# iosefa/obia

Hardware: AMD Instinct MI355X
Metric: Mpixel/s (SLIC+zonal feats) on 16384²×8-band; achieved HBM GB/s fraction (higher is better)
Workload: dtype f32

## Files before the change

### obia_amd/_lib.py

```python
import ctypes
import os
import subprocess

import numpy as np

_CSRC = os.path.join(os.path.dirname(os.path.abspath(__file__)), "csrc")
LIB_PATH = os.environ.get("OBIA_HIP_LIB") or os.path.join(_CSRC, "libobia_hip.so")

OBIA_OK = 0
MASK_SEEDS_CHUNK = 1024
E_INVALID, E_HIP, E_NOMEM, E_UNSUPPORTED, E_EMPTY, E_NONFINITE = -1, -2, -3, -4, -5, -6


class SlicParams(ctypes.Structure):
    _fields_ = [("compactness", ctypes.c_double), ("min_size_factor", ctypes.c_double),
                ("max_size_factor", ctypes.c_double), ("n_segments", ctypes.c_int32),
                ("max_num_iter", ctypes.c_int32), ("convert2lab", ctypes.c_int32),
                ("enforce_connectivity", ctypes.c_int32), ("slic_zero", ctypes.c_int32),
                ("start_label", ctypes.c_int32), ("normalize_bands", ctypes.c_int32),
                ("exit_on_fixed_point", ctypes.c_int32), ("reserved", ctypes.c_int32),
                ("sigma_zyx", ctypes.c_double * 3), ("spacing_zyx", ctypes.c_double * 3)]


class SlicSeeds(ctypes.Structure):
# ... 159 lines not shown


def last_error():
    return load().obia_last_error().decode("utf-8", "replace")


def check(rc):
    if rc == OBIA_OK:
        return
    msg = last_error()
    if rc in (E_INVALID, E_EMPTY, E_NONFINITE):
        raise ValueError(msg)
    if rc == E_UNSUPPORTED:
        raise NotImplementedError(msg)
    if rc == E_NOMEM:
        raise MemoryError(msg)
    raise RuntimeError(f"obia_hip error {rc}: {msg}")


class Context:

    def __init__(self, device=0, stream=None):
        lib = load()
        if stream is None:
            self._h = lib.obia_create(int(device))
        else:
            self._h = lib.obia_create_on_stream(int(device), ctypes.c_void_p(int(stream)))
        if not self._h:
            raise RuntimeError(f"obia_create failed: {last_error()} (obia_amd needs an AMD GPU; there is no CPU path)")
        self.device = int(device)

    @property
    def handle(self):
        return self._h

    def close(self):
        if getattr(self, "_h", None):
            load().obia_destroy(self._h)
            self._h = None

    def __del__(self):
        try:
            self.close()
        except Exception:
            pass

    def set_profiling(self, on):
        check(load().obia_set_profiling(self._h, int(on)))

    def timing(self):
        lib = load()
        names = ["assign_ms", "sweeps", "features_ms", "connectivity_ms", "zonal_ms", "total_ms", "prepass_ms", "assign_px",
                 "prepass_px", "assign_store_px", "assign_busy_ms", "prepass_busy_ms", "batch_repeats",
                 "prepass_shared_px", "feature_fused_px", "prepass_group_launches", "fills", "uploads", "readbacks"]
        return {n: lib.obia_last_timing(self._h, i) for i, n in enumerate(names)}

    def workspace_bytes(self):
        return int(load().obia_workspace_bytes(self._h))


_default_ctx = {}


def default_context(device=0):
    ctx = _default_ctx.get(device)
    if ctx is None:
        ctx = _default_ctx[device] = Context(device)
    return ctx


def np_ptr(a):
    return None if a is None else ctypes.c_void_p(a.ctypes.data)


def mask_bytes(mask, device=None):
    import torch
    m = torch.as_tensor(mask, device=device)
    if m.dtype == torch.bool:
        m = m.contiguous().view(torch.uint8)
    elif m.dtype != torch.uint8:
        m = (m != 0).view(torch.uint8)
    return m.contiguous()
```

### obia_amd/csrc/common.hpp

```cpp
#pragma once
#include <hip/hip_runtime.h>
#include <algorithm>
#include <cstdint>
#include <cstdio>
#include <cstring>
#include <string>
#include <vector>

#include "../../include/obia_hip.h"

struct obia_ctx;

namespace obia {

void set_error(const char *fmt, ...);

#define OBIA_HIP_TRY(expr)                                                                       \
    do {                                                                                         \
        hipError_t e__ = (expr);                                                                 \
        if (e__ != hipSuccess) {                                                                 \
            obia::set_error("%s:%d: %s -> %s", __FILE__, __LINE__, #expr, hipGetErrorString(e__)); \
            return OBIA_E_HIP;                                                                   \
        }                                                                                        \
    } while (0)

#define OBIA_TRY(expr)            \
    do {                          \
        int rc__ = (expr);        \
        if (rc__ != OBIA_OK) return rc__; \
    } while (0)

class Arena {
  public:
    ~Arena() { release(); }
    void *alloc(size_t bytes);
    template <typename T> T *get(size_t n) { return static_cast<T *>(alloc(n * sizeof(T))); }
    void reset();
    void release();
    struct Mark { size_t block, used, total; };
    Mark mark() const;
    void rewind(const Mark &m);
    size_t capacity() const;
    bool failed() const { return failed_; }

  private:
    struct Block { char *p; size_t size; size_t used; };
    std::vector<Block> blocks_;
    size_t high_water_ = 0, cur_total_ = 0, cur_ = 0;
    bool failed_ = false;
};

class PlanBlob {
  public:
    template <typename T> T *add(obia_ctx *ctx, const T *host, size_t n) { return static_cast<T *>(add_bytes(ctx, host, n * sizeof(T))); }
    int flush(obia_ctx *ctx);
    void drop() { dev_ = host_ = nullptr; cap_ = used_ = 0; }
  private:
    void *add_bytes(obia_ctx *ctx, const void *host, size_t bytes);
    char *dev_ = nullptr, *host_ = nullptr;
    size_t cap_ = 0, used_ = 0;
};

struct Timing {
    double assign_ms = 0, prepass_ms = 0, feat_ms = 0, cc_ms = 0, zonal_ms = 0, total_ms = 0;
    double assign_px = 0, prepass_px = 0;
    double prepass_shared_px = 0;
    double assign_store_px = 0;
    double feat_fused_px = 0;
    int sweeps = 0;
    int prepass_group_launches = 0;
    int batch_repeats = 0;
    double assign_busy_ms = 0, prepass_busy_ms = 0;
    int fills = 0, uploads = 0, readbacks = 0;
};

}

struct obia_ctx {
    int device = 0;
    hipStream_t stream = nullptr;
    bool own_stream = false;
    obia::Arena arena;
    void *pinned = nullptr;
    size_t pinned_bytes = 0;
    unsigned long long *defer_buf = nullptr;
    bool defer_pending = false;
    double defer_shared_px = 0;
    int32_t *cc_visited = nullptr;
    size_t cc_visited_px = 0;
    bool cc_visited_dirty = false;
    char *up_buf = nullptr;
    size_t up_bytes = 0, up_used = 0;
    obia::PlanBlob plan;
    int profiling = 0;
    obia::Timing timing;
    struct Span { int kind; hipEvent_t a, b; };
    std::vector<Span> spans;
    std::vector<hipEvent_t> event_pool;
    size_t events_used = 0;
    hipStream_t side = nullptr;
    hipEvent_t aux_fork = nullptr, aux_join = nullptr;
    hipEvent_t grp_fork = nullptr, grp_join = nullptr;
    int spatial_residency[4] = {0, 0, 0, 0};
};

namespace obia {

enum TimeKind { T_ASSIGN = 0, T_FEAT = 2, T_CC = 3, T_ZONAL = 4, T_TOTAL = 5, T_PREPASS = 6 };

struct ScopedSpan {
    obia_ctx *ctx; bool on; size_t idx;
    ScopedSpan(obia_ctx *c, int kind);
    ~ScopedSpan();
};
struct KernelSpan {
    hipEvent_t a = nullptr, b = nullptr;
    KernelSpan(obia_ctx *c, int kind);
};
void begin_timing(obia_ctx *ctx);
void resolve_timing(obia_ctx *ctx);

int read_back(obia_ctx *ctx, void *host_dst, const void *dev_src, size_t bytes);
int upload_async(obia_ctx *ctx, void *dev_dst, const void *host_src, size_t bytes);
int fill_async(obia_ctx *ctx, void *dev_dst, int byte, size_t bytes);

struct ClearRange { void *p; unsigned long long bytes; unsigned value, pad; };
struct ClearTable { ClearRange r[16]; int n; };
class ClearSet {
  public:
    explicit ClearSet(obia_ctx *ctx) : ctx_(ctx) { t_.n = 0; }
    int add(void *dev, int byte, size_t bytes);
    int flush();
  private:
    obia_ctx *ctx_;
    ClearTable t_;
};

int side_stream(obia_ctx *ctx);
void debug_sync(obia_ctx *ctx, const char *stage);

static inline int cdiv(long long a, long long b) { return (int)((a + b - 1) / b); }
static inline unsigned flat_grid(long long n) { return (unsigned)std::max<long long>(1, std::min<long long>(cdiv(n, 256), 8192)); }


int enter(obia_ctx *ctx);

int quiesce(obia_ctx *ctx, int rc);

enum FrameOpts : unsigned { FRAME_PLAIN = 0, FRAME_TIMING = 1, FRAME_TOTAL = 2 | FRAME_TIMING };
void frame_begin(obia_ctx *ctx, unsigned opts);
int frame_end(obia_ctx *ctx, unsigned opts, int rc);
template <typename Body> int call_frame(obia_ctx *ctx, unsigned opts, Body &&body) {
    frame_begin(ctx, opts);
    int rc;
    if ((opts & FRAME_TOTAL) == FRAME_TOTAL) {
        ScopedSpan total(ctx, T_TOTAL);
        rc = body();
    } else {
        rc = body();
    }
    return frame_end(ctx, opts, rc);
}

class Staging {
  public:
    explicit Staging(obia_ctx *ctx) : ctx_(ctx) {}
    ~Staging() { (void)finish(); }
    Staging(const Staging &) = delete;
    Staging &operator=(const Staging &) = delete;
    template <typename T> T *in(const T *host, size_t n) { return static_cast<T *>(upload(host, n * sizeof(T))); }
// ... 25 lines not shown
```

### obia_amd/csrc/context.cpp

```cpp
#include "common.hpp"
#include "../../include/obia_testing.h"

#include <algorithm>
#include <cstdlib>
#include <utility>

#include <cstdarg>

namespace obia {

static thread_local std::string g_last_error;

void set_error(const char *fmt, ...) {
    char buf[1024];
    va_list ap;
    va_start(ap, fmt);
    vsnprintf(buf, sizeof(buf), fmt, ap);
    va_end(ap);
    g_last_error = buf;
}

void *Arena::alloc(size_t bytes) {
    bytes = (bytes + 255) & ~size_t(255);
    if (bytes == 0) bytes = 256;
// ... 49 lines not shown
    if (blocks_.size() > 1) {
        size_t total = 0;
        for (auto &b : blocks_) total += b.size;
        for (auto &b : blocks_) (void)hipFree(b.p);
        blocks_.clear();
        void *p = nullptr;
        if (hipMalloc(&p, high_water_ + (high_water_ >> 3)) == hipSuccess) blocks_.push_back(Block{static_cast<char *>(p), high_water_ + (high_water_ >> 3), 0});
        (void)total;
    } else if (!blocks_.empty()) {
        blocks_[0].used = 0;
    }
}

void Arena::release() {
    for (auto &b : blocks_) (void)hipFree(b.p);
    blocks_.clear();
}

size_t Arena::capacity() const {
    size_t t = 0;
    for (auto &b : blocks_) t += b.size;
    return t;
}

static hipEvent_t get_event(obia_ctx *ctx) {
    if (ctx->events_used == ctx->event_pool.size()) {
        hipEvent_t e = nullptr;
        (void)hipEventCreate(&e);
        ctx->event_pool.push_back(e);
    }
    return ctx->event_pool[ctx->events_used++];
}

ScopedSpan::ScopedSpan(obia_ctx *c, int kind) : ctx(c), on(c->profiling == 1 || (c->profiling == 2 && kind == T_ASSIGN)), idx(0) {
    if (!on) return;
    obia_ctx::Span s{kind, get_event(ctx), get_event(ctx)};
    (void)hipEventRecord(s.a, ctx->stream);
    idx = ctx->spans.size();
    ctx->spans.push_back(s);
}
ScopedSpan::~ScopedSpan() {
    if (on) (void)hipEventRecord(ctx->spans[idx].b, ctx->stream);
}

int side_stream(obia_ctx *ctx) {
    if (!ctx->aux_fork) OBIA_HIP_TRY(hipEventCreateWithFlags(&ctx->aux_fork, hipEventDisableTiming));
    if (!ctx->aux_join) OBIA_HIP_TRY(hipEventCreateWithFlags(&ctx->aux_join, hipEventDisableTiming));
    if (!ctx->grp_fork) OBIA_HIP_TRY(hipEventCreateWithFlags(&ctx->grp_fork, hipEventDisableTiming));
    if (!ctx->grp_join) OBIA_HIP_TRY(hipEventCreateWithFlags(&ctx->grp_join, hipEventDisableTiming));
    if (!ctx->side) OBIA_HIP_TRY(hipStreamCreateWithFlags(&ctx->side, hipStreamNonBlocking));
    return OBIA_OK;
}

KernelSpan::KernelSpan(obia_ctx *c, int kind) {
    if (!(c->profiling == 1 || (c->profiling == 2 && kind == T_ASSIGN))) return;
    a = get_event(c);
    b = get_event(c);
    c->spans.push_back(obia_ctx::Span{kind, a, b});
}

void begin_timing(obia_ctx *ctx) {
    ctx->spans.clear();
    ctx->events_used = 0;
    ctx->timing = Timing();
}

void resolve_timing(obia_ctx *ctx) {
    if (!ctx->profiling) return;
    (void)hipStreamSynchronize(ctx->stream);
    std::vector<std::pair<double, double>> iv[2];
    hipEvent_t ref = nullptr;
    for (auto &s : ctx->spans) {
        float ms = 0;
        if (hipEventElapsedTime(&ms, s.a, s.b) != hipSuccess) { (void)hipGetLastError(); continue; }
        if (s.kind == T_ASSIGN || s.kind == T_PREPASS) {
            if (!ref) ref = s.a;
            float end = 0;
            if (hipEventElapsedTime(&end, ref, s.b) == hipSuccess) iv[s.kind == T_ASSIGN ? 0 : 1].emplace_back((double)end - ms, (double)end);
            else (void)hipGetLastError();
        }
        switch (s.kind) {
            case T_ASSIGN: ctx->timing.assign_ms += ms; ctx->timing.sweeps += 1; break;
            case T_FEAT: ctx->timing.feat_ms += ms; break;
            case T_CC: ctx->timing.cc_ms += ms; break;
            case T_ZONAL: ctx->timing.zonal_ms += ms; break;
            case T_TOTAL: ctx->timing.total_ms += ms; break;
            case T_PREPASS: ctx->timing.prepass_ms += ms; break;
            default: break;
        }
    }
    for (int c = 0; c < 2; ++c) {
        std::sort(iv[c].begin(), iv[c].end());
        double busy = 0, lo = 0, hi = -1;
        for (auto &x : iv[c]) {
            if (hi < lo || x.first > hi) { if (hi > lo) busy += hi - lo; lo = x.first; hi = x.second; }
            else if (x.second > hi) hi = x.second;
        }
        if (hi > lo) busy += hi - lo;
        (c == 0 ? ctx->timing.assign_busy_ms : ctx->timing.prepass_busy_ms) += busy;
    }
    ctx->spans.clear();
}

int read_back(obia_ctx *ctx, void *host_dst, const void *dev_src, size_t bytes) {
    if (bytes > ctx->pinned_bytes) {
        if (ctx->pinned) (void)hipHostFree(ctx->pinned);
        ctx->pinned = nullptr;
        size_t want = bytes < 4096 ? 4096 : bytes;
        OBIA_HIP_TRY(hipHostMalloc(&ctx->pinned, want, hipHostMallocDefault));
        ctx->pinned_bytes = want;
    }
    OBIA_TRY(ctx->plan.flush(ctx));
    OBIA_HIP_TRY(hipMemcpyAsync(ctx->pinned, dev_src, bytes, hipMemcpyDeviceToHost, ctx->stream));
    ctx->timing.readbacks += 1;
    OBIA_HIP_TRY(hipStreamSynchronize(ctx->stream));
    ctx->up_used = 0;
    memcpy(host_dst, ctx->pinned, bytes);
    return OBIA_OK;
}

void debug_sync(obia_ctx *ctx, const char *stage) {
    static const bool on = std::getenv("OBIA_DEBUG_SYNC") != nullptr;
    if (!on) return;
    const hipError_t e = hipStreamSynchronize(ctx->stream);
    fprintf(stderr, "[obia debug] %s: %s\n", stage, e == hipSuccess ? "ok" : hipGetErrorString(e));
    fflush(stderr);
}

int fill_async(obia_ctx *ctx, void *dev_dst, int byte, size_t bytes) {
    if (bytes == 0) return OBIA_OK;
    OBIA_HIP_TRY(hipMemsetAsync(dev_dst, byte, bytes, ctx->stream));
    ctx->timing.fills += 1;
    return OBIA_OK;
}

template <bool RAGGED> __global__ __launch_bounds__(256) void clear_ranges_kernel(const ClearTable T) {
    const size_t tid = (size_t)blockIdx.x * blockDim.x + threadIdx.x, stride = (size_t)gridDim.x * blockDim.x;
    for (int k = 0; k < T.n; ++k) {
        unsigned char *p = static_cast<unsigned char *>(T.r[k].p);
        const size_t n = T.r[k].bytes;
        const unsigned v = (T.r[k].value & 0xffu) * 0x01010101u;
        size_t head = RAGGED ? (16 - (reinterpret_cast<uintptr_t>(p) & 15)) & 15 : 0;
        if (head > n) head = n;
        const size_t nvec = (n - head) / 16, tail0 = head + nvec * 16;
        uint4 *pv = reinterpret_cast<uint4 *>(p + head);
        for (size_t i = tid; i < nvec; i += stride) pv[i] = make_uint4(v, v, v, v);
        if (RAGGED) {
            if (tid < head) p[tid] = (unsigned char)v;
            if (tid < n - tail0) p[tail0 + tid] = (unsigned char)v;
        }
    }
}

// ... 245 lines not shown
        for (int i = 0; i < n; ++i) OBIA_TRY(clr.add(dev_ptrs[i], values[i], (size_t)bytes[i]));
        return clr.flush();
    });
}

int64_t obia_workspace_bytes(obia_ctx *ctx) { return ctx ? (int64_t)ctx->arena.capacity() : 0; }

void obia_slic_default_params(obia_slic_params *p) {
    if (!p) return;
    p->n_segments = 100;
    p->compactness = 10.0;
    p->max_num_iter = 10;
    p->convert2lab = -1;
    p->enforce_connectivity = 1;
    p->min_size_factor = 0.5;
    p->max_size_factor = 3.0;
    p->slic_zero = 0;
    p->start_label = 1;
    p->normalize_bands = 0;
    p->exit_on_fixed_point = 0;
    p->reserved = 0;
    p->sigma_zyx[0] = p->sigma_zyx[1] = p->sigma_zyx[2] = 0.0;
    p->spacing_zyx[0] = p->spacing_zyx[1] = p->spacing_zyx[2] = 1.0;
}

int obia_set_profiling(obia_ctx *ctx, int enabled) {
    if (!ctx) { set_error("null context"); return OBIA_E_INVALID; }
    ctx->profiling = enabled < 0 ? 0 : (enabled > 2 ? 1 : enabled);
    return OBIA_OK;
}

double obia_last_timing(obia_ctx *ctx, int what) {
    if (!ctx) return -1.0;
    switch (what) {
        case 0: return ctx->timing.assign_ms;
        case 1: return (double)ctx->timing.sweeps;
        case 2: return ctx->timing.feat_ms;
        case 3: return ctx->timing.cc_ms;
        case 4: return ctx->timing.zonal_ms;
        case 5: return ctx->timing.total_ms;
        case 6: return ctx->timing.prepass_ms;
        case 7: return ctx->timing.assign_px;
        case 8: return ctx->timing.prepass_px;
        case 9: return ctx->timing.assign_store_px;
        case 10: return ctx->timing.assign_busy_ms;
        case 11: return ctx->timing.prepass_busy_ms;
        case 12: return (double)ctx->timing.batch_repeats;
        case 13: return ctx->timing.prepass_shared_px;
        case 14: return ctx->timing.feat_fused_px;
        case 15: return (double)ctx->timing.prepass_group_launches;
        case 16: return (double)ctx->timing.fills;
        case 17: return (double)ctx->timing.uploads;
        case 18: return (double)ctx->timing.readbacks;
        default: return -1.0;
    }
}

}
```

### obia_amd/csrc/slic_sweep.hip

```cpp
#include "slic.hpp"
#include "slic_features.hpp"

#include <type_traits>
#include <hip/hip_ext.h>

#include <cstdlib>

namespace obia {

#ifdef OBIA_STAMP
__device__ unsigned long long g_tl[65536 * 4 * 24];
#define STAMP_DECL unsigned long long st_t = clock64(), st_t0 = st_t, st_r0 = __builtin_amdgcn_s_memrealtime(), st_acc[12] = {0, 0, 0, 0, 0, 0, 0, 0, 0, 0, 0, 0}, st_cnt[6] = {0, 0, 0, 0, 0, 0};
#define STAMP_COUNT(i, v) st_cnt[i] += (v);
#define STAMP(i) { const unsigned long long st_n = clock64(); st_acc[i] += st_n - st_t; st_t = st_n; }
#ifndef OBIA_STAMP_KIND
#define OBIA_STAMP_KIND 0
#endif
#define STAMP_FLUSH if (accumulate && (LEAN ? 1 : 0) == OBIA_STAMP_KIND && (threadIdx.x & 63) == 0 && gtile < 65536) { unsigned long long *st_o = g_tl + ((size_t)gtile * 4 + (threadIdx.x >> 6)) * 24; for (int st_i = 0; st_i < 12; ++st_i) st_o[st_i] = st_acc[st_i]; st_o[12] = st_t0; st_o[13] = clock64(); st_o[14] = st_r0; st_o[15] = __builtin_amdgcn_s_memrealtime(); for (int st_i = 0; st_i < 6; ++st_i) st_o[16 + st_i] = st_cnt[st_i]; }
#else
#define STAMP_DECL
#define STAMP(i)
#define STAMP_COUNT(i, v)
#define STAMP_FLUSH
#endif
// ... 1096 lines not shown
    slic_assign_body<CP, MASKED, false, false, false, false, true, NCH>(OBIA_ASSIGN_ARGS, nullptr);
}

template <int CP, bool MASKED, bool FIXPT>
__global__ __launch_bounds__(NT) __attribute__((amdgpu_waves_per_eu(LEAN_WAVES, LEAN_WAVES))) void slic_prepass_kernel(OBIA_ASSIGN_PARAMS, const int *__restrict__ act_tiles) {
    slic_assign_body<CP, MASKED, true, FIXPT, false, true, false>(OBIA_ASSIGN_ARGS, act_tiles);
}

#include "slic_spatial.hip"

#ifdef OBIA_STAMP
extern "C" void obia_debug_timeline(unsigned long long *out, int nwaves) {
    (void)hipMemcpyFromSymbol(out, HIP_SYMBOL(g_tl), sizeof(unsigned long long) * 24 * (size_t)nwaves);
}
#endif

template <int CP, bool MASKED>
__global__ __launch_bounds__(256) void slic_maxdist_kernel(const SlicProblem *__restrict__ probs, const float *__restrict__ feat,
                                                           const uint8_t *__restrict__ mask, const int32_t *__restrict__ labels,
                                                           float *__restrict__ cent, int start_label, int nch) {
    constexpr int RS = CENT_REC + CP;
    const SlicProblem P = probs[blockIdx.y];
    for (int y = blockIdx.x; y < P.H; y += gridDim.x)
        for (int x = threadIdx.x; x < P.W; x += 256) {
            const long long pix = P.pix_off + (long long)y * P.W + x;
            if (MASKED && mask[pix] == 0) continue;
            const int l = labels[pix];
            if (l < start_label) continue;
            const int k = l - start_label + P.cent_off;
            const float *rec = cent + (size_t)k * RS;
            float dc = 0.0f;
#pragma unroll
            for (int ch = 0; ch < CP; ++ch) {
                if (ch >= nch) break;
                const float t = feat_at(feat, P, CP, y, x, ch) - rec[CENT_REC + ch];
                dc += t * t;
            }
            unsigned *slot = reinterpret_cast<unsigned *>(cent + (size_t)k * RS + 7);
            if (__float_as_uint(dc) > __hip_atomic_load(slot, __ATOMIC_RELAXED, __HIP_MEMORY_SCOPE_AGENT)) atomicMax(slot, __float_as_uint(dc));
        }
}

struct TileSubset { const int *table = nullptr; int base = 0, end = -1; };

struct FixedPointState {
    int *bin_stamp = nullptr, *tile_lp = nullptr, *cache_k = nullptr;
    unsigned long long *cache_q = nullptr;
};

template <int CP>
static void launch_assign(obia_ctx *ctx, SlicBatch &b, int ignore_color, int accumulate, int accum_color, int store_labels,
                          int *orphan_flag, const FixedPointState &fp, int sweep_id, int use_cache, unsigned long long *px_counter,
                          const KernelSpan &span, const int *head_cur, bool prepass_visits, const TileSubset &sub = TileSubset(),
                          bool rawin = false, const hipStream_t *on = nullptr) {
    const hipStream_t stream = on ? *on : ctx->stream;
    constexpr int XGH = OBIA_XCD_GROUP;
    const int ntiles = sub.end >= 0 ? sub.end : (int)b.total_tiles_all, tbase = sub.end >= 0 ? sub.base : 0;
    dim3 grid(8 * XGH * (unsigned)((ntiles - tbase + 8 * XGH - 1) / (8 * XGH)));
    const int RQ = acc_record_qwords(CP);
    int tpp = b.probs.empty() ? 0 : b.probs[0].tiles_x * b.probs[0].tiles_y;
    for (auto &P : b.probs) if (P.tiles_x * P.tiles_y != tpp) tpp = 0;
#define LAUNCH_ARGS_                                                                                                 \
    b.d_probs, b.d_feat, b.d_mask, b.d_mask4, b.d_cent, head_cur, b.d_labels, b.d_acc, RQ, accumulate, store_labels, b.start_label,      \
        (float)b.fscale, fp.bin_stamp, fp.tile_lp, fp.cache_k, fp.cache_q, sweep_id, use_cache, px_counter,          \
        b.d_tile_prob, ntiles, orphan_flag, tpp, b.d_fbox, tbase, b.C, b.d_tl_k, b.d_tl_fp, b.d_tl_meta, b.d_tl_req
#define LAUNCH_K_(...)                                                                                               \
    hipExtLaunchKernelGGL(HIP_KERNEL_NAME(__VA_ARGS__), grid, dim3(NT), 0, stream, span.a, span.b, 0, LAUNCH_ARGS_)
#define LAUNCH_KL_(...)                                                                                              \
    hipExtLaunchKernelGGL(HIP_KERNEL_NAME(__VA_ARGS__), grid, dim3(NT), 0, stream, span.a, span.b, 0, LAUNCH_ARGS_, sub.table)
    const int pad = CP - b.C;
    if constexpr (CP <= 12) if (rawin) {
        RawInput ri;
        ri.src = b.raw_src; ri.Ws = b.raw_ws; ri.wins = b.d_windows; ri.keys = b.d_keys; ri.ratio = b.feat_ratio; ri.planes = b.d_feat;
        hipExtLaunchKernelGGL(HIP_KERNEL_NAME(slic_assign_rawin_kernel<CP>), grid, dim3(NT), 0, stream, span.a, span.b, 0, LAUNCH_ARGS_, ri);
        ctx->timing.feat_fused_px += (double)b.total_pix;
        return;
    }
#define LAUNCH_ASSIGN_(M, I, F, Z) LAUNCH_K_(slic_assign_kernel<CP, M, I, F, Z>)
#define LAUNCH_MAIN_(M)                                                                                              \
    do {                                                                                                             \
        if (pad == 1) LAUNCH_K_(slic_assign_kernel<CP, M, false, false, false, CP - 1>);                             \
        else if (pad == 2) LAUNCH_K_(slic_assign_kernel<CP, M, false, false, false, CP - 2>);                        \
        else if (pad == 3) LAUNCH_K_(slic_assign_kernel<CP, M, false, false, false, CP - 3>);                        \
        else LAUNCH_K_(slic_assign_kernel<CP, M, false, false, false>);                                              \
    } while (0)
#define LAUNCH_COLLB_(M)                                                                                             \
    do {                                                                                                             \
        if (pad == 1) LAUNCH_K_(slic_assign_collb_kernel<CP, M, CP - 1>);                                            \
        else if (pad == 2) LAUNCH_K_(slic_assign_collb_kernel<CP, M, CP - 2>);                                       \
        else if (pad == 3) LAUNCH_K_(slic_assign_collb_kernel<CP, M, CP - 3>);                                       \
        else LAUNCH_K_(slic_assign_collb_kernel<CP, M>);                                                             \
    } while (0)
#define LAUNCH_LEAN_(M, F) LAUNCH_KL_(slic_prepass_kernel<CP, M, F>)
#define LAUNCH_ASSIGN(M, I)                                                                                          \
    do {                                                                                                             \
        if ((I) && !accum_color) {                                                                                   \
            if (fp.bin_stamp) LAUNCH_LEAN_(M, true);                                                                 \
            else if (store_labels || prepass_visits) LAUNCH_LEAN_(M, false);                                         \
            else LAUNCH_KL_(slic_spatial_kernel<CP>);                                                                \
        }                                                                                                            \
        else if (b.slic_zero && !(I)) LAUNCH_ASSIGN_(M, false, false, true);                                         \
        else if (fp.bin_stamp) LAUNCH_ASSIGN_(M, I, true, false);                                                    \
        else if (b.col_lb && b.d_fbox && !(I)) LAUNCH_COLLB_(M);                                                     \
        else if (!(I)) LAUNCH_MAIN_(M);                                                                              \
        else LAUNCH_ASSIGN_(M, I, false, false);                                                                     \
    } while (0)
    if (b.masked) { if (ignore_color) LAUNCH_ASSIGN(true, true); else LAUNCH_ASSIGN(true, false); }
    else LAUNCH_ASSIGN(false, false);
#undef LAUNCH_ASSIGN
#undef LAUNCH_ASSIGN_
#undef LAUNCH_LEAN_
#undef LAUNCH_COLLB_
#undef LAUNCH_MAIN_
#undef LAUNCH_K_
#undef LAUNCH_KL_
#undef LAUNCH_ARGS_
}

__global__ __launch_bounds__(256) void mask_pack4_kernel(const SlicProblem *__restrict__ probs, const uint8_t *__restrict__ mask,
                                                         unsigned *__restrict__ mask4) {
    const SlicProblem P = probs[blockIdx.y];
    if ((long long)P.n_valid == (long long)P.H * (long long)P.W) return;
    const int nq = (P.H + 3) >> 2, W = P.W;
// ... 25 lines not shown
            for (int x = threadIdx.x; x < W; x += 256) {
                unsigned w = 0u;
#pragma unroll
                for (int j = 0; j < 4; ++j) {
                    const int y = 4 * q + j;
                    if (y < P.H) w |= (unsigned)(mb[(long long)y * W + x] != 0) << (8 * j);
                }
                out[(long long)q * W + x] = w;
            }
        }
    }
}

__global__ void fill_i32_kernel(int32_t *p, long long n, int32_t v) {
    for (long long i = (long long)blockIdx.x * blockDim.x + threadIdx.x; i < n; i += (long long)gridDim.x * blockDim.x) p[i] = v;
}

static void fill_labels(obia_ctx *ctx, SlicBatch &b) {
    const long long n = b.total_pix;
    int blocks = cdiv(n, 256 * 8);
    if (blocks > 65535) blocks = 65535;
    if (blocks < 1) blocks = 1;
    hipLaunchKernelGGL(fill_i32_kernel, dim3(blocks), dim3(256), 0, ctx->stream, b.d_labels, n, b.start_label - 1);
}

static void fold_counters(obia_ctx *ctx, const unsigned long long *h, double shared_px) {
    if (ctx->profiling) {
        for (int i = 0; i < 256; ++i) { ctx->timing.assign_px += (double)h[i]; ctx->timing.prepass_px += (double)h[256 + i]; }
        ctx->timing.prepass_px += shared_px;
        ctx->timing.prepass_shared_px += shared_px;
    }
}

static int spatial_residency(obia_ctx *ctx, int CP) {
    int &r = ctx->spatial_residency[CP / 4 - 1];
    if (r > 0) return r;
    int per_cu = 0, cus = 0;
    hipError_t e = hipErrorInvalidValue;
    switch (CP) {
        case 8: e = hipOccupancyMaxActiveBlocksPerMultiprocessor(&per_cu, slic_spatial_kernel<8>, NT, 0); break;
#ifndef OBIA_ONLY_CP8
        case 4: e = hipOccupancyMaxActiveBlocksPerMultiprocessor(&per_cu, slic_spatial_kernel<4>, NT, 0); break;
        case 12: e = hipOccupancyMaxActiveBlocksPerMultiprocessor(&per_cu, slic_spatial_kernel<12>, NT, 0); break;
        case 16: e = hipOccupancyMaxActiveBlocksPerMultiprocessor(&per_cu, slic_spatial_kernel<16>, NT, 0); break;
#endif
        default: break;
    }
    if (e == hipSuccess) e = hipDeviceGetAttribute(&cus, hipDeviceAttributeMultiprocessorCount, ctx->device);
    if (e != hipSuccess || per_cu <= 0 || cus <= 0) { (void)hipGetLastError(); return 0x7fffffff; }
    r = per_cu * cus;
    return r;
}

static int queue_sweeps(obia_ctx *ctx, SlicBatch &b, bool repeat, unsigned long long **d_px_out, double *shared_px_out) {
    *d_px_out = nullptr;
    *shared_px_out = 0.0;
    if (std::getenv("OBIA_DEBUG_SYNC"))
        for (size_t p = 0; p < b.probs.size(); ++p) {
            const SlicProblem &P = b.probs[p];
            fprintf(stderr, "[obia debug]   problem %zu: %dx%d K %d steps %d %d bins %dx%d cell_off %d cent_off %d tiles %dx%d tile_off %d n_valid %d (total_cent %d total_cells %d tiles_all %lld)\n",
                    p, P.H, P.W, P.K, P.sy, P.sx, P.ncy, P.ncx, P.cell_off, P.cent_off, P.tiles_y, P.tiles_x, P.tile_off, P.n_valid,
                    b.total_cent, b.total_cells, b.total_tiles_all);
        }
    if (b.total_tiles <= 0 || b.max_iter <= 0) { fill_labels(ctx, b); return OBIA_OK; }
    for (auto &P : b.probs)
        if (P.W >= (1 << 22)) { set_error("rasters / tile windows wider than 4194303 pixels are not supported (got %d)", P.W); return OBIA_E_UNSUPPORTED; }
    const int passes = (b.masked && !b.prepass_only) ? 2 : 1;
    if (b.fuse_features && (!b.masked || b.exit_on_fixed_point || b.slic_zero || b.direct || b.col_lb || b.C != b.CP || b.CP > 12 || !b.raw_src || !b.d_keys)) {
        set_error("fused feature pass on a batch that cannot take it");
        return OBIA_E_INVALID;
    }
    const int pre_iter = (b.masked && b.prepass_iter > 0) ? b.prepass_iter : b.max_iter;
    const int total_sweeps = b.masked ? pre_iter + (passes - 1) * b.max_iter : b.max_iter;
    const int RQ = acc_record_qwords(b.CP);
    Arena &A = ctx->arena;
    unsigned long long *d_px = A.get<unsigned long long>(513);
    if (!d_px) return OBIA_E_NOMEM;
    int *d_orphan = reinterpret_cast<int *>(d_px + 512);
    FixedPointState fp;
    if (b.exit_on_fixed_point) {
        const size_t nt = (size_t)b.total_tiles_all;
        fp.bin_stamp = A.get<int>((size_t)b.total_cells);
        fp.tile_lp = A.get<int>(nt);
        fp.cache_k = A.get<int>(nt * (MAXC + 1));
        fp.cache_q = A.get<unsigned long long>(nt * MAXC * (size_t)(b.CP + 3));
        if (!fp.bin_stamp || !fp.tile_lp || !fp.cache_k || !fp.cache_q) return OBIA_E_NOMEM;
        OBIA_TRY(fill_async(ctx, fp.bin_stamp, 0, sizeof(int) * (size_t)b.total_cells));
        OBIA_TRY(fill_async(ctx, fp.tile_lp, 0, sizeof(int) * nt));
    }
    {
        const size_t nt = (size_t)b.total_tiles_all;
        b.d_tl_k = A.get<int>(nt * MAXC);
        b.d_tl_fp = A.get<unsigned>(nt * NT);
        b.d_tl_meta = A.get<int>(nt * 3);
        b.d_tl_req = b.d_tl_meta ? b.d_tl_meta + nt * 2 : nullptr;
        b.d_ref = A.get<float>((size_t)b.total_cent * 2);
        if (!b.d_tl_k || !b.d_tl_fp || !b.d_tl_meta || !b.d_tl_req || !b.d_ref) return OBIA_E_NOMEM;
    }
    int maxh_z = 1, kmax = 1;
    for (auto &P : b.probs) { if (P.H > maxh_z) maxh_z = P.H; if (P.K > kmax) kmax = P.K; }
    if (b.masked && b.d_mask && !b.d_mask4) {
        b.d_mask4 = A.get<unsigned>((size_t)b.total_m4);
        if (!b.d_mask4) return OBIA_E_NOMEM;
        int gq = (maxh_z + 3) / 4;
        if (gq > 16384) gq = 16384;
        OBIA_TRY(ctx->plan.flush(ctx));
// ... 3 lines not shown

    const bool store_all = repeat || b.exit_on_fixed_point || b.slic_zero;
    if (store_all || total_sweeps <= 1) {
        fill_labels(ctx, b);
        debug_sync(ctx, "sweeps: label fill");
    }
    const bool prep_grouped = std::getenv("OBIA_PREP_GROUPED") != nullptr;
    const bool prepass_visits = std::getenv("OBIA_PREPASS_VISITS") != nullptr;
    std::vector<int> share_rep;
    int n_shared = 0;
    {
        const char *e = std::getenv("OBIA_PREPASS_SHARE");
        const bool off = e && e[0] == '0';
        if (!off && b.masked && passes == 2 && pre_iter >= 2 && b.prepass_iter <= 0 && !store_all && !b.direct && !prep_grouped)
            n_shared = slic_prepass_classes(b.probs, b.grid_n, share_rep);
    }
    TileSubset act_tiles;
    const int *d_act_probs = nullptr;
    const int *d_member_rep = nullptr;
    int act_p_base = 0, n_act = b.nprob, kmax_act = kmax, kmax_mem = 1;
    if (n_shared > 0) {
        std::vector<int> ap, at, mr;
        double spx = 0.0;
        kmax_act = 1;
        for (int p = 0; p < b.nprob; ++p) {
            const SlicProblem &P = b.probs[p];
            if (share_rep[p] == p) {
                ap.push_back(p);
                for (int t = 0; t < P.tiles_x * P.tiles_y; ++t) at.push_back(P.tile_off + t);
                if (P.K > kmax_act) kmax_act = P.K;
            } else {
                mr.push_back(p); mr.push_back(share_rep[p]);
                if (P.K > kmax_mem) kmax_mem = P.K;
                spx += (double)P.H * (double)P.W * (double)(pre_iter - 1);
            }
        }
        n_act = (int)ap.size();
        act_p_base = ap.front();
        const bool span = ap.back() - ap.front() + 1 == n_act;
        d_member_rep = ctx->plan.add(ctx, mr.data(), mr.size());
        if (!d_member_rep) return OBIA_E_NOMEM;
        if (span) {
            act_tiles.base = b.probs[ap.front()].tile_off;
            act_tiles.end = b.probs[ap.back()].tile_off + b.probs[ap.back()].tiles_x * b.probs[ap.back()].tiles_y;
        } else {
            const int *d_ap = ctx->plan.add(ctx, ap.data(), ap.size()), *d_at = ctx->plan.add(ctx, at.data(), at.size());
            if (!d_ap || !d_at) return OBIA_E_NOMEM;
            d_act_probs = d_ap;
            act_tiles.table = d_at; act_tiles.base = 0; act_tiles.end = (int)at.size();
        }
        *shared_px_out = spx;
    }
    int grp_split = 0;
    {
        const char *e = std::getenv("OBIA_PREPASS_GROUPS");
        const int mode = !e ? 1 : (e[0] == '0' ? 0 : (e[0] == '2' ? 2 : 1));
        if (mode != 0 && n_shared == 0 && b.masked && pre_iter >= 2 && !store_all && !prepass_visits && !prep_grouped && !b.direct &&
            b.nprob >= 2 && !std::getenv("OBIA_DEBUG_SYNC")) {
            long long best = -1;
            for (int p = 1; p < b.nprob; ++p) {
                const long long t0 = b.probs[p].tile_off, t1 = b.total_tiles_all - t0, d = t0 > t1 ? t0 - t1 : t1 - t0;
                if (t0 > 0 && t1 > 0 && (best < 0 || d <= best)) { best = d; grp_split = p; }
            }
            if (grp_split > 0 && mode != 2) {
                const long long t0 = b.probs[grp_split].tile_off, t1 = b.total_tiles_all - t0;
                if ((t0 < t1 ? t0 : t1) < (long long)spatial_residency(ctx, b.CP)) grp_split = 0;
            }
            if (grp_split > 0) OBIA_TRY(side_stream(ctx));
        }
    }
    OBIA_TRY(ctx->plan.flush(ctx));
    {
        ClearSet clr(ctx);
        OBIA_TRY(clr.add(b.d_acc, 0, sizeof(unsigned long long) * (size_t)b.total_cent * RQ));
        OBIA_TRY(clr.add(d_px, 0, sizeof(unsigned long long) * 513));
        OBIA_TRY(clr.add(b.d_head, 0xff, sizeof(int) * (size_t)b.total_cells));
        OBIA_TRY(clr.add(b.d_tl_meta, 0xff, sizeof(int) * 3 * (size_t)b.total_tiles_all));
        OBIA_TRY(clr.flush());
    }
    debug_sync(ctx, "sweeps: memsets");
    bool first = true;
    int sweep_no = 0;
    for (int pass = 0; pass < passes; ++pass) {
        const int ignore_color = (b.masked && pass == 0) ? 1 : 0;
        const bool last_pass = (pass == passes - 1);
        if (pass > 0 && store_all) {
            fill_labels(ctx, b);
            if (fp.tile_lp) OBIA_TRY(fill_async(ctx, fp.tile_lp, 0, sizeof(int) * (size_t)b.total_tiles_all));
        }
        const int iters = ignore_color ? pre_iter : b.max_iter;
        for (int it = 0; it < iters; ++it) {
            int *head_cur = b.d_head + (size_t)(sweep_no & 1) * b.total_cells;
            int *head_nxt = b.d_head + (size_t)((sweep_no + 1) & 1) * b.total_cells;
            ++sweep_no;
            const int zmode = (b.slic_zero && !ignore_color) ? (it == 0 ? 2 : 1) : 0;
            const bool shared_sweep = n_shared > 0 && ignore_color && it < iters - 1;
            if (n_shared > 0 && ignore_color && it == iters - 1) {
                hipLaunchKernelGGL(slic_prepass_broadcast_kernel, dim3(cdiv(kmax_mem, 64), n_shared), dim3(64), 0, ctx->stream, b.d_probs,
                                   d_member_rep, b.CP, RQ, b.d_acc, b.d_cent, b.d_ref);
                debug_sync(ctx, "sweeps: pre-pass broadcast");
            }
            const dim3 prep_grid(cdiv(shared_sweep ? kmax_act : kmax, 64), shared_sweep ? n_act : b.nprob);
            const int prep_base = shared_sweep ? act_p_base : 0;
            const int *prep_table = shared_sweep ? d_act_probs : nullptr;
#define LAUNCH_PREP_LANE(CPV)                                                                                         \
    hipLaunchKernelGGL(HIP_KERNEL_NAME(slic_prep_lane_kernel<CPV>), pgrid, dim3(64), 0, stream, \
                       b.d_probs, p_base, first ? 1 : 0, zmode, b.d_seed, b.d_acc, RQ, 1.0 / b.fscale, b.d_cent, head_cur, head_nxt, \
                       cell_end, fp.bin_stamp, sweep_no, cell_base, b.d_ref, b.d_tl_req, table)
            auto prep_lane = [&](hipStream_t stream, dim3 pgrid, int p_base, const int *table, int cell_base, int cell_end) {
                switch (b.CP) {
                    case 4: LAUNCH_PREP_LANE(4); break;
                    case 8: LAUNCH_PREP_LANE(8); break;
                    case 12: LAUNCH_PREP_LANE(12); break;
                    default: LAUNCH_PREP_LANE(16); break;
                }
            };
#undef LAUNCH_PREP_LANE
            if (grp_split > 0 && ignore_color && it < iters - 1) {
                hipError_t he = hipSuccess;
                if (it == 0) {
                    he = hipEventRecord(ctx->grp_fork, ctx->stream);
                    if (he == hipSuccess) he = hipStreamWaitEvent(ctx->side, ctx->grp_fork, 0);
                }
                for (int g = 0; g < 2 && he == hipSuccess; ++g) {
                    const int p0 = g ? grp_split : 0, p1 = g ? b.nprob : grp_split;
                    int kmax_g = 1;
                    for (int p = p0; p < p1; ++p) if (b.probs[p].K > kmax_g) kmax_g = b.probs[p].K;
                    const hipStream_t st = g ? ctx->side : ctx->stream;
                    prep_lane(st, dim3(cdiv(kmax_g, 64), p1 - p0), p0, nullptr, b.probs[p0].cell_off, g ? b.total_cells : b.probs[p1].cell_off);
                    KernelSpan span(ctx, T_PREPASS);
                    TileSubset sub;
                    sub.base = b.probs[p0].tile_off;
                    sub.end = g ? (int)b.total_tiles_all : b.probs[p1].tile_off;
                    unsigned long long *pxc = ctx->profiling ? d_px + 256 : nullptr;
                    switch (b.CP) {
                        case 8: launch_assign<8>(ctx, b, 1, 1, 0, 0, d_orphan, fp, sweep_no, 1, pxc, span, head_cur, false, sub, false, &st); break;
#ifndef OBIA_ONLY_CP8
                        case 4: launch_assign<4>(ctx, b, 1, 1, 0, 0, d_orphan, fp, sweep_no, 1, pxc, span, head_cur, false, sub, false, &st); break;
                        case 12: launch_assign<12>(ctx, b, 1, 1, 0, 0, d_orphan, fp, sweep_no, 1, pxc, span, head_cur, false, sub, false, &st); break;
                        case 16: launch_assign<16>(ctx, b, 1, 1, 0, 0, d_orphan, fp, sweep_no, 1, pxc, span, head_cur, false, sub, false, &st); break;
#endif
                        default: he = hipErrorInvalidValue; break;
                    }
                    ctx->timing.prepass_group_launches += 1;
                }
                if (he == hipSuccess && it == iters - 2) {
                    he = hipEventRecord(ctx->grp_join, ctx->side);
                    if (he == hipSuccess) he = hipStreamWaitEvent(ctx->stream, ctx->grp_join, 0);
                }
                if (he != hipSuccess) {
                    (void)hipStreamSynchronize(ctx->side);
                    set_error("grouped pre-pass: %s", hipGetErrorString(he));
                    return OBIA_E_HIP;
                }
                b.d_head_cur = head_cur;
                first = false;
                continue;
            }
            if (!prep_grouped) prep_lane(ctx->stream, prep_grid, prep_base, prep_table, 0, b.total_cells);
            else if (RQ == 16)
                hipLaunchKernelGGL(HIP_KERNEL_NAME(slic_prep_kernel<16>), dim3(cdiv(b.total_cent * 16LL, 256)), dim3(256), 0,
                                   ctx->stream, b.d_probs, b.d_cent_prob, b.total_cent, b.CP, first ? 1 : 0, zmode, b.d_seed, b.d_acc,
                                   1.0 / b.fscale, b.d_cent, head_cur, head_nxt, b.total_cells, fp.bin_stamp, sweep_no, 0, 0, b.d_ref, b.d_tl_req);
            else
                hipLaunchKernelGGL(HIP_KERNEL_NAME(slic_prep_kernel<32>), dim3(cdiv(b.total_cent * 32LL, 256)), dim3(256), 0,
                                   ctx->stream, b.d_probs, b.d_cent_prob, b.total_cent, b.CP, first ? 1 : 0, zmode, b.d_seed, b.d_acc,
                                   1.0 / b.fscale, b.d_cent, head_cur, head_nxt, b.total_cells, fp.bin_stamp, sweep_no, 0, 0, b.d_ref, b.d_tl_req);
            b.d_head_cur = head_cur;
            debug_sync(ctx, "sweeps: prep");
            first = false;
            if (zmode == 1) {
                dim3 zg(maxh_z, b.nprob);
#define LAUNCH_MAXDIST(CPV)                                                                                           \
    do {                                                                                                              \
        if (b.masked) hipLaunchKernelGGL(HIP_KERNEL_NAME(slic_maxdist_kernel<CPV, true>), zg, dim3(256), 0, ctx->stream, b.d_probs, \
                                         b.d_feat, b.d_mask, b.d_labels, b.d_cent, b.start_label, b.C);            \
        else hipLaunchKernelGGL(HIP_KERNEL_NAME(slic_maxdist_kernel<CPV, false>), zg, dim3(256), 0, ctx->stream, b.d_probs, \
                                b.d_feat, b.d_mask, b.d_labels, b.d_cent, b.start_label, b.C);                     \
    } while (0)
                switch (b.CP) {
                    case 4: LAUNCH_MAXDIST(4); break;
                    case 8: LAUNCH_MAXDIST(8); break;
                    case 12: LAUNCH_MAXDIST(12); break;
                    default: LAUNCH_MAXDIST(16); break;
                }
#undef LAUNCH_MAXDIST
            }
            const bool very_last = last_pass && it == iters - 1;
            const int accumulate = very_last ? 0 : 1;
            const int accum_color = (!ignore_color || it == iters - 1) ? 1 : 0;
            const int store_labels = store_all ? 2 : (very_last ? 1 : 0);
            const int use_cache = (ignore_color && it == iters - 1) ? 0 : 1;
            const bool rawin = b.fuse_features && !repeat && ignore_color && it == iters - 1;
            {
                KernelSpan span(ctx, ignore_color ? T_PREPASS : T_ASSIGN);
                const TileSubset sub = shared_sweep ? act_tiles : TileSubset();
                unsigned long long *pxc = ctx->profiling ? d_px + (ignore_color ? 256 : 0) : nullptr;
                if (ctx->profiling && !ignore_color && store_labels) ctx->timing.assign_store_px += (double)b.total_pix;
                switch (b.CP) {
                    case 8: launch_assign<8>(ctx, b, ignore_color, accumulate, accum_color, store_labels, d_orphan, fp, sweep_no, use_cache, pxc, span, head_cur, prepass_visits, sub, rawin); break;
#ifndef OBIA_ONLY_CP8
                    case 4: launch_assign<4>(ctx, b, ignore_color, accumulate, accum_color, store_labels, d_orphan, fp, sweep_no, use_cache, pxc, span, head_cur, prepass_visits, sub, rawin); break;
                    case 12: launch_assign<12>(ctx, b, ignore_color, accumulate, accum_color, store_labels, d_orphan, fp, sweep_no, use_cache, pxc, span, head_cur, prepass_visits, sub, rawin); break;
                    case 16: launch_assign<16>(ctx, b, ignore_color, accumulate, accum_color, store_labels, d_orphan, fp, sweep_no, use_cache, pxc, span, head_cur, prepass_visits, sub); break;
#endif
// ... 48 lines not shown
```

Baseline: 7559.

## Split colour-pass assign sweeps into two problem groups on parallel streams

Extends the existing grouped pre-pass scheme to the full colour sweeps. Problems are split into two halves by tile count, and each half's prep and assign kernels run on the main and side streams, joined only at the end of the sweep chain. This removes the per-sweep serialisation across problems, so the two halves can progress independently and fill the GPU better. The split is gated on each half having at least an occupancy-derived residency's worth of tiles, computed with a new occupancy query path. Profiling accounting is extended for the grouped launches. The risk is extra launches and contention between the two streams.

```diff
diff --git a/obia_amd/_lib.py b/obia_amd/_lib.py
--- a/obia_amd/_lib.py
+++ b/obia_amd/_lib.py
@@ -235,7 +235,8 @@
         lib = load()
         names = ["assign_ms", "sweeps", "features_ms", "connectivity_ms", "zonal_ms", "total_ms", "prepass_ms", "assign_px",
                  "prepass_px", "assign_store_px", "assign_busy_ms", "prepass_busy_ms", "batch_repeats",
-                 "prepass_shared_px", "feature_fused_px", "prepass_group_launches", "fills", "uploads", "readbacks"]
+                 "prepass_shared_px", "feature_fused_px", "prepass_group_launches", "fills", "uploads", "readbacks",
+                 "assign_group_launches", "assign_launch_sum_ms"]
         return {n: lib.obia_last_timing(self._h, i) for i, n in enumerate(names)}
 
     def workspace_bytes(self):
diff --git a/obia_amd/csrc/common.hpp b/obia_amd/csrc/common.hpp
--- a/obia_amd/csrc/common.hpp
+++ b/obia_amd/csrc/common.hpp
@@ -69,6 +69,9 @@
     double feat_fused_px = 0;
     int sweeps = 0;
     int prepass_group_launches = 0;
+    int assign_group_launches = 0;
+    int assign_group_batches = 0;
+    double assign_launch_sum_ms = 0;
     int batch_repeats = 0;
     double assign_busy_ms = 0, prepass_busy_ms = 0;
     int fills = 0, uploads = 0, readbacks = 0;
@@ -94,7 +97,7 @@
     obia::PlanBlob plan;
     int profiling = 0;
     obia::Timing timing;
-    struct Span { int kind; hipEvent_t a, b; };
+    struct Span { int kind; hipEvent_t a, b; int tag = 0; };
     std::vector<Span> spans;
     std::vector<hipEvent_t> event_pool;
     size_t events_used = 0;
@@ -102,11 +105,12 @@
     hipEvent_t aux_fork = nullptr, aux_join = nullptr;
     hipEvent_t grp_fork = nullptr, grp_join = nullptr;
     int spatial_residency[4] = {0, 0, 0, 0};
+    int sweep_residency[64] = {};
 };
 
 namespace obia {
 
-enum TimeKind { T_ASSIGN = 0, T_FEAT = 2, T_CC = 3, T_ZONAL = 4, T_TOTAL = 5, T_PREPASS = 6 };
+enum TimeKind { T_ASSIGN = 0, T_FEAT = 2, T_CC = 3, T_ZONAL = 4, T_TOTAL = 5, T_PREPASS = 6, T_ASSIGN_GRP = 7 };
 
 struct ScopedSpan {
     obia_ctx *ctx; bool on; size_t idx;
@@ -115,7 +119,8 @@
 };
 struct KernelSpan {
     hipEvent_t a = nullptr, b = nullptr;
-    KernelSpan(obia_ctx *c, int kind);
+    KernelSpan() = default;
+    KernelSpan(obia_ctx *c, int kind, int tag = 0);
 };
 void begin_timing(obia_ctx *ctx);
 void resolve_timing(obia_ctx *ctx);
diff --git a/obia_amd/csrc/context.cpp b/obia_amd/csrc/context.cpp
--- a/obia_amd/csrc/context.cpp
+++ b/obia_amd/csrc/context.cpp
@@ -125,11 +125,11 @@
     return OBIA_OK;
 }
 
-KernelSpan::KernelSpan(obia_ctx *c, int kind) {
-    if (!(c->profiling == 1 || (c->profiling == 2 && kind == T_ASSIGN))) return;
+KernelSpan::KernelSpan(obia_ctx *c, int kind, int tag) {
+    if (!(c->profiling == 1 || (c->profiling == 2 && (kind == T_ASSIGN || kind == T_ASSIGN_GRP)))) return;
     a = get_event(c);
     b = get_event(c);
-    c->spans.push_back(obia_ctx::Span{kind, a, b});
+    c->spans.push_back(obia_ctx::Span{kind, a, b, tag});
 }
 
 void begin_timing(obia_ctx *ctx) {
@@ -141,19 +141,40 @@
 void resolve_timing(obia_ctx *ctx) {
     if (!ctx->profiling) return;
     (void)hipStreamSynchronize(ctx->stream);
-    std::vector<std::pair<double, double>> iv[2];
+    typedef std::vector<std::pair<double, double>> Intervals;
+    auto union_ms = [](Intervals &v) {
+        std::sort(v.begin(), v.end());
+        double busy = 0, lo = 0, hi = -1;
+        for (auto &x : v) {
+            if (hi < lo || x.first > hi) { if (hi > lo) busy += hi - lo; lo = x.first; hi = x.second; }
+            else if (x.second > hi) hi = x.second;
+        }
+        if (hi > lo) busy += hi - lo;
+        return busy;
+    };
+    Intervals iv[2];
+    std::vector<Intervals> grouped;
     hipEvent_t ref = nullptr;
     for (auto &s : ctx->spans) {
         float ms = 0;
         if (hipEventElapsedTime(&ms, s.a, s.b) != hipSuccess) { (void)hipGetLastError(); continue; }
-        if (s.kind == T_ASSIGN || s.kind == T_PREPASS) {
+        if (s.kind == T_ASSIGN || s.kind == T_ASSIGN_GRP || s.kind == T_PREPASS) {
             if (!ref) ref = s.a;
             float end = 0;
-            if (hipEventElapsedTime(&end, ref, s.b) == hipSuccess) iv[s.kind == T_ASSIGN ? 0 : 1].emplace_back((double)end - ms, (double)end);
+            if (hipEventElapsedTime(&end, ref, s.b) == hipSuccess) {
+                const std::pair<double, double> x((double)end - ms, (double)end);
+                iv[s.kind == T_PREPASS ? 1 : 0].push_back(x);
+                if (s.kind == T_ASSIGN_GRP) {
+                    const size_t batch = (size_t)(s.tag >> 1);
+                    if (grouped.size() <= batch) grouped.resize(batch + 1);
+                    grouped[batch].push_back(x);
+                }
+            }
             else (void)hipGetLastError();
         }
         switch (s.kind) {
-            case T_ASSIGN: ctx->timing.assign_ms += ms; ctx->timing.sweeps += 1; break;
+            case T_ASSIGN: ctx->timing.assign_ms += ms; ctx->timing.assign_launch_sum_ms += ms; ctx->timing.sweeps += 1; break;
+            case T_ASSIGN_GRP: ctx->timing.assign_launch_sum_ms += ms; if (!(s.tag & 1)) ctx->timing.sweeps += 1; break;
             case T_FEAT: ctx->timing.feat_ms += ms; break;
             case T_CC: ctx->timing.cc_ms += ms; break;
             case T_ZONAL: ctx->timing.zonal_ms += ms; break;
@@ -162,16 +183,9 @@
             default: break;
         }
     }
-    for (int c = 0; c < 2; ++c) {
-        std::sort(iv[c].begin(), iv[c].end());
-        double busy = 0, lo = 0, hi = -1;
-        for (auto &x : iv[c]) {
-            if (hi < lo || x.first > hi) { if (hi > lo) busy += hi - lo; lo = x.first; hi = x.second; }
-            else if (x.second > hi) hi = x.second;
-        }
-        if (hi > lo) busy += hi - lo;
-        (c == 0 ? ctx->timing.assign_busy_ms : ctx->timing.prepass_busy_ms) += busy;
-    }
+    for (auto &g : grouped) ctx->timing.assign_ms += union_ms(g);
+    ctx->timing.assign_busy_ms += union_ms(iv[0]);
+    ctx->timing.prepass_busy_ms += union_ms(iv[1]);
     ctx->spans.clear();
 }
 
@@ -523,6 +537,8 @@
         case 16: return (double)ctx->timing.fills;
         case 17: return (double)ctx->timing.uploads;
         case 18: return (double)ctx->timing.readbacks;
+        case 19: return (double)ctx->timing.assign_group_launches;
+        case 20: return ctx->timing.assign_launch_sum_ms;
         default: return -1.0;
     }
 }
diff --git a/obia_amd/csrc/slic_sweep.hip b/obia_amd/csrc/slic_sweep.hip
--- a/obia_amd/csrc/slic_sweep.hip
+++ b/obia_amd/csrc/slic_sweep.hip
@@ -1172,7 +1172,7 @@
 static void launch_assign(obia_ctx *ctx, SlicBatch &b, int ignore_color, int accumulate, int accum_color, int store_labels,
                           int *orphan_flag, const FixedPointState &fp, int sweep_id, int use_cache, unsigned long long *px_counter,
                           const KernelSpan &span, const int *head_cur, bool prepass_visits, const TileSubset &sub = TileSubset(),
-                          bool rawin = false, const hipStream_t *on = nullptr) {
+                          bool rawin = false, const hipStream_t *on = nullptr, int *occupancy = nullptr) {
     const hipStream_t stream = on ? *on : ctx->stream;
     constexpr int XGH = OBIA_XCD_GROUP;
     const int ntiles = sub.end >= 0 ? sub.end : (int)b.total_tiles_all, tbase = sub.end >= 0 ? sub.base : 0;
@@ -1185,10 +1185,14 @@
         (float)b.fscale, fp.bin_stamp, fp.tile_lp, fp.cache_k, fp.cache_q, sweep_id, use_cache, px_counter,          \
         b.d_tile_prob, ntiles, orphan_flag, tpp, b.d_fbox, tbase, b.C, b.d_tl_k, b.d_tl_fp, b.d_tl_meta, b.d_tl_req
 #define LAUNCH_K_(...)                                                                                               \
-    hipExtLaunchKernelGGL(HIP_KERNEL_NAME(__VA_ARGS__), grid, dim3(NT), 0, stream, span.a, span.b, 0, LAUNCH_ARGS_)
+    do {                                                                                                             \
+        if (!occupancy) hipExtLaunchKernelGGL(HIP_KERNEL_NAME(__VA_ARGS__), grid, dim3(NT), 0, stream, span.a, span.b, 0, LAUNCH_ARGS_); \
+        else if (hipOccupancyMaxActiveBlocksPerMultiprocessor(occupancy, __VA_ARGS__, NT, 0) != hipSuccess) { (void)hipGetLastError(); *occupancy = 0; } \
+    } while (0)
 #define LAUNCH_KL_(...)                                                                                              \
     hipExtLaunchKernelGGL(HIP_KERNEL_NAME(__VA_ARGS__), grid, dim3(NT), 0, stream, span.a, span.b, 0, LAUNCH_ARGS_, sub.table)
     const int pad = CP - b.C;
+    if (occupancy && (rawin || ignore_color)) { *occupancy = 0; return; }
     if constexpr (CP <= 12) if (rawin) {
         RawInput ri;
         ri.src = b.raw_src; ri.Ws = b.raw_ws; ri.wins = b.d_windows; ri.keys = b.d_keys; ri.ratio = b.feat_ratio; ri.planes = b.d_feat;
@@ -1320,6 +1324,48 @@
     return r;
 }
 
+static int sweep_residency(obia_ctx *ctx, SlicBatch &b) {
+    const bool collb = b.col_lb && b.d_fbox;
+    int &r = ctx->sweep_residency[(((b.CP / 4 - 1) * 2 + (b.masked ? 1 : 0)) * 4 + (b.CP - b.C)) * 2 + (collb ? 1 : 0)];
+    if (r > 0) return r;
+    int per_cu = 0, cus = 0;
+    const FixedPointState fp;
+    const KernelSpan span;
+    switch (b.CP) {
+        case 8: launch_assign<8>(ctx, b, 0, 1, 1, 0, nullptr, fp, 0, 1, nullptr, span, nullptr, false, TileSubset(), false, nullptr, &per_cu); break;
+#ifndef OBIA_ONLY_CP8
+        case 4: launch_assign<4>(ctx, b, 0, 1, 1, 0, nullptr, fp, 0, 1, nullptr, span, nullptr, false, TileSubset(), false, nullptr, &per_cu); break;
+        case 12: launch_assign<12>(ctx, b, 0, 1, 1, 0, nullptr, fp, 0, 1, nullptr, span, nullptr, false, TileSubset(), false, nullptr, &per_cu); break;
+        case 16: launch_assign<16>(ctx, b, 0, 1, 1, 0, nullptr, fp, 0, 1, nullptr, span, nullptr, false, TileSubset(), false, nullptr, &per_cu); break;
+#endif
+        default: break;
+    }
+    if (per_cu <= 0 || hipDeviceGetAttribute(&cus, hipDeviceAttributeMultiprocessorCount, ctx->device) != hipSuccess || cus <= 0) {
+        (void)hipGetLastError();
+        return 0x7fffffff;
+    }
+    r = per_cu * cus;
+    return r;
+}
+
+static int group_split(const SlicBatch &b) {
+    int split = 0;
+    long long best = -1;
+    for (int p = 1; p < b.nprob; ++p) {
+        const long long t0 = b.probs[p].tile_off, t1 = b.total_tiles_all - t0, d = t0 > t1 ? t0 - t1 : t1 - t0;
+        if (t0 > 0 && t1 > 0 && (best < 0 || d <= best)) { best = d; split = p; }
+    }
+    return split;
+}
+static long long group_min_tiles(const SlicBatch &b, int split) {
+    const long long t0 = b.probs[split].tile_off, t1 = b.total_tiles_all - t0;
+    return t0 < t1 ? t0 : t1;
+}
+static int groups_mode(const char *name) {
+    const char *e = std::getenv(name);
+    return !e ? 1 : (e[0] == '0' ? 0 : (e[0] == '2' ? 2 : 1));
+}
+
 static int queue_sweeps(obia_ctx *ctx, SlicBatch &b, bool repeat, unsigned long long **d_px_out, double *shared_px_out) {
     *d_px_out = nullptr;
     *shared_px_out = 0.0;
@@ -1429,22 +1475,18 @@
         *shared_px_out = spx;
     }
     int grp_split = 0;
-    {
-        const char *e = std::getenv("OBIA_PREPASS_GROUPS");
-        const int mode = !e ? 1 : (e[0] == '0' ? 0 : (e[0] == '2' ? 2 : 1));
-        if (mode != 0 && n_shared == 0 && b.masked && pre_iter >= 2 && !store_all && !prepass_visits && !prep_grouped && !b.direct &&
-            b.nprob >= 2 && !std::getenv("OBIA_DEBUG_SYNC")) {
-            long long best = -1;
-            for (int p = 1; p < b.nprob; ++p) {
-                const long long t0 = b.probs[p].tile_off, t1 = b.total_tiles_all - t0, d = t0 > t1 ? t0 - t1 : t1 - t0;
-                if (t0 > 0 && t1 > 0 && (best < 0 || d <= best)) { best = d; grp_split = p; }
-            }
-            if (grp_split > 0 && mode != 2) {
-                const long long t0 = b.probs[grp_split].tile_off, t1 = b.total_tiles_all - t0;
-                if ((t0 < t1 ? t0 : t1) < (long long)spatial_residency(ctx, b.CP)) grp_split = 0;
-            }
-            if (grp_split > 0) OBIA_TRY(side_stream(ctx));
-        }
+    int col_split = 0;
+    if (!store_all && !prepass_visits && !prep_grouped && !b.direct && b.nprob >= 2 &&
+        !std::getenv("OBIA_DEBUG_SYNC")) {
+        const int split = group_split(b);
+        const int pre_mode = groups_mode("OBIA_PREPASS_GROUPS"), col_mode = groups_mode("OBIA_SWEEP_GROUPS");
+        if (split > 0 && pre_mode != 0 && n_shared == 0 && b.masked && pre_iter >= 2 &&
+            (pre_mode == 2 || group_min_tiles(b, split) >= (long long)spatial_residency(ctx, b.CP)))
+            grp_split = split;
+        if (split > 0 && col_mode != 0 && !(b.masked && b.prepass_only) && b.max_iter >= 2 &&
+            (col_mode == 2 || group_min_tiles(b, split) >= (long long)sweep_residency(ctx, b)))
+            col_split = split;
+        if (grp_split > 0 || col_split > 0) OBIA_TRY(side_stream(ctx));
     }
     OBIA_TRY(ctx->plan.flush(ctx));
     {
@@ -1493,41 +1535,47 @@
                 }
             };
 #undef LAUNCH_PREP_LANE
-            if (grp_split > 0 && ignore_color && it < iters - 1) {
+            const bool pre_groups = grp_split > 0 && ignore_color && it < iters - 1, col_groups = col_split > 0 && !ignore_color;
+            if (pre_groups || col_groups) {
+                const int split = col_groups ? col_split : grp_split;
+                const bool chain_end = it == (col_groups ? iters - 1 : iters - 2), very_last = col_groups && chain_end;
                 hipError_t he = hipSuccess;
                 if (it == 0) {
                     he = hipEventRecord(ctx->grp_fork, ctx->stream);
                     if (he == hipSuccess) he = hipStreamWaitEvent(ctx->side, ctx->grp_fork, 0);
+                    if (col_groups) ctx->timing.assign_group_batches += 1;
                 }
                 for (int g = 0; g < 2 && he == hipSuccess; ++g) {
-                    const int p0 = g ? grp_split : 0, p1 = g ? b.nprob : grp_split;
+                    const int p0 = g ? split : 0, p1 = g ? b.nprob : split;
                     int kmax_g = 1;
                     for (int p = p0; p < p1; ++p) if (b.probs[p].K > kmax_g) kmax_g = b.probs[p].K;
                     const hipStream_t st = g ? ctx->side : ctx->stream;
                     prep_lane(st, dim3(cdiv(kmax_g, 64), p1 - p0), p0, nullptr, b.probs[p0].cell_off, g ? b.total_cells : b.probs[p1].cell_off);
-                    KernelSpan span(ctx, T_PREPASS);
+                    KernelSpan span(ctx, col_groups ? T_ASSIGN_GRP : T_PREPASS, col_groups ? 2 * (ctx->timing.assign_group_batches - 1) + g : 0);
                     TileSubset sub;
                     sub.base = b.probs[p0].tile_off;
                     sub.end = g ? (int)b.total_tiles_all : b.probs[p1].tile_off;
-                    unsigned long long *pxc = ctx->profiling ? d_px + 256 : nullptr;
+                    unsigned long long *pxc = ctx->profiling ? d_px + (col_groups ? 0 : 256) : nullptr;
+                    const int ign = col_groups ? 0 : 1, accumulate = very_last ? 0 : 1, store_labels = very_last ? 1 : 0;
                     switch (b.CP) {
-                        case 8: launch_assign<8>(ctx, b, 1, 1, 0, 0, d_orphan, fp, sweep_no, 1, pxc, span, head_cur, false, sub, false, &st); break;
+                        case 8: launch_assign<8>(ctx, b, ign, accumulate, 1 - ign, store_labels, d_orphan, fp, sweep_no, 1, pxc, span, head_cur, false, sub, false, &st); break;
 #ifndef OBIA_ONLY_CP8
-                        case 4: launch_assign<4>(ctx, b, 1, 1, 0, 0, d_orphan, fp, sweep_no, 1, pxc, span, head_cur, false, sub, false, &st); break;
-                        case 12: launch_assign<12>(ctx, b, 1, 1, 0, 0, d_orphan, fp, sweep_no, 1, pxc, span, head_cur, false, sub, false, &st); break;
-                        case 16: launch_assign<16>(ctx, b, 1, 1, 0, 0, d_orphan, fp, sweep_no, 1, pxc, span, head_cur, false, sub, false, &st); break;
+                        case 4: launch_assign<4>(ctx, b, ign, accumulate, 1 - ign, store_labels, d_orphan, fp, sweep_no, 1, pxc, span, head_cur, false, sub, false, &st); break;
+                        case 12: launch_assign<12>(ctx, b, ign, accumulate, 1 - ign, store_labels, d_orphan, fp, sweep_no, 1, pxc, span, head_cur, false, sub, false, &st); break;
+                        case 16: launch_assign<16>(ctx, b, ign, accumulate, 1 - ign, store_labels, d_orphan, fp, sweep_no, 1, pxc, span, head_cur, false, sub, false, &st); break;
 #endif
                         default: he = hipErrorInvalidValue; break;
                     }
-                    ctx->timing.prepass_group_launches += 1;
-                }
-                if (he == hipSuccess && it == iters - 2) {
+                    (col_groups ? ctx->timing.assign_group_launches : ctx->timing.prepass_group_launches) += 1;
+                }
+                if (very_last && ctx->profiling) ctx->timing.assign_store_px += (double)b.total_pix;
+                if (he == hipSuccess && chain_end) {
                     he = hipEventRecord(ctx->grp_join, ctx->side);
                     if (he == hipSuccess) he = hipStreamWaitEvent(ctx->stream, ctx->grp_join, 0);
                 }
                 if (he != hipSuccess) {
                     (void)hipStreamSynchronize(ctx->side);
-                    set_error("grouped pre-pass: %s", hipGetErrorString(he));
+                    set_error("grouped %s: %s", col_groups ? "colour pass" : "pre-pass", hipGetErrorString(he));
                     return OBIA_E_HIP;
                 }
                 b.d_head_cur = head_cur;
```

New measurement: 7729 (median of 6 runs). 1.02x the previous value.
